# brownvc/matryodshka

Measured on AMD Instinct MI355X. Metric: novel-view frames/sec, 640x320 ODS->32-sphere MSI infer+render, higher is better.
Workload: dtype f32

## Files before the change

### matryodshka_amd/csrc/cnn_x3.hip

```cpp
#include "cnn_device.h"

namespace {

#ifndef MSI_X3_EARLY_DMA
#define MSI_X3_EARLY_DMA 0
#endif
#ifndef MSI_X3_NSTG
#define MSI_X3_NSTG 0
#endif
#ifndef MSI_X3_ABLATE
#define MSI_X3_ABLATE 0
#endif
#ifndef MSI_X2_NSTG
#define MSI_X2_NSTG 3
#endif
constexpr int x3_rate_y(int RATE) { return RATE == 3 ? 1 : RATE; }
constexpr int x3_rate_x(int RATE) { return RATE == 3 ? 2 : RATE; }
constexpr int x3_nstg(int RATE, int NPL) { return NPL == 2 ? MSI_X2_NSTG : (MSI_X3_NSTG ? MSI_X3_NSTG : (RATE == 2 ? 3 : 2)); }
template <int RATE, int NS = x3_nstg(RATE, 3), int NPL = 3, int TH = 4>
struct HaloGeomX3 {
  static constexpr int PW = 16 + 2 * x3_rate_x(RATE), PH = TH + 2 * x3_rate_y(RATE), NPX = PW * PH;
  static constexpr int PIX_BYTES = NPL * 64 + 16;
  static constexpr int ROW_PITCH = ((PW * PIX_BYTES + 127) / 256) * 256 + 128;
  static constexpr int A_BYTES = PH * ROW_PITCH;
  static constexpr int B_ROW = 64;
  static constexpr int B_PLANE = 64 * B_ROW, B_STAGE = NPL * B_PLANE;
  static constexpr int NSTG = NS;
  static constexpr int LDS_BYTES = A_BYTES + NSTG * B_STAGE;
  static constexpr int NLOAD = (NPX * 8 + 255) / 256;
};
__device__ __forceinline__ void f16_range_track(unsigned &amax, v4f y) {
  const float fx = y.x, fy = y.y, fz = y.z, fw = y.w;
  const unsigned a = __builtin_bit_cast(unsigned, fx) & 0x7fffffffu, b = __builtin_bit_cast(unsigned, fy) & 0x7fffffffu;
  const unsigned c = __builtin_bit_cast(unsigned, fz) & 0x7fffffffu, d = __builtin_bit_cast(unsigned, fw) & 0x7fffffffu;
  amax = max(max(amax, a), max(b, max(c, d)));
}
constexpr unsigned F16_MAX_BITS = 0x477fe000u;

template <int N>
__device__ __forceinline__ void wait_lgkm4(v4f &a, v4f &b, v4f &c, v4f &d) {
  asm volatile("s_waitcnt lgkmcnt(%4)" : "+v"(a), "+v"(b), "+v"(c), "+v"(d) : "n"(N) : "memory");
}
template <int N>
__device__ __forceinline__ void wait_lgkm6(v4f &a, v4f &b, v4f &c, v4f &d, v4f &e, v4f &f) {
  asm volatile("s_waitcnt lgkmcnt(%6)" : "+v"(a), "+v"(b), "+v"(c), "+v"(d), "+v"(e), "+v"(f) : "n"(N) : "memory");
}

#ifndef MSI_X2_WAVES
#define MSI_X2_WAVES 4
#endif
#ifndef MSI_X2_LATE_CB
#define MSI_X2_LATE_CB 1
#endif
template <int NP>
__device__ __forceinline__ void split_mfma(f32x16 &acc, f32x16 &lo, const v4f &ah, const v4f &am, const v4f &al, const v4f &bh, const v4f &bm, const v4f &bl);
template <int RATE, int APPLY, int NPL, int TH>
__device__ __forceinline__ void conv_halo_x3_body(const ConvParams &p, char *smem) {
  typedef HaloGeomX3<RATE, x3_nstg(RATE, NPL), NPL, TH> G;
  constexpr int RY = x3_rate_y(RATE), RX = x3_rate_x(RATE), PW = G::PW, NPX = G::NPX, NLOAD = G::NLOAD;
  static_assert(RATE != 3 || TH == 4, "row-parity tiles: four rows");
  constexpr int MT = TH / 4, NT = 1, BM = 16 * TH;
  static_assert(TH == 4 || (TH == 8 && NPL == 3 && RATE == 1), "the 8-row tile is built for the six-product form at rate 1");
#ifdef MSI_CONV_TIMING
  const unsigned long long ts0 = __builtin_amdgcn_s_memtime(), ts0r = __builtin_amdgcn_s_memrealtime();
#endif
  const int tid = threadIdx.x, lane = tid & 63;
  const int wave = __builtin_amdgcn_readfirstlane(tid >> 6);
  const int wm = wave >> 1, wn = wave & 1;
  const int CH = p.cpt0;
  int t, c0 = 0, c1 = CH, ks = 0, slot = 0;
  {
    const int bid = blockIdx.x;
    if (bid < p.nb_main && p.split0 == 1) {
      const int q = p.n_main >> 3, r = p.n_main & 7, xcd = bid & 7, local = bid >> 3;
      t = (xcd < r ? xcd * (q + 1) : r * (q + 1) + (xcd - r) * q) + local;
    } else {
      int sp, r, tbase;
      unsigned mg;
      if (bid < p.nb_main) { sp = p.split0; mg = p.mg_sp0; r = bid; tbase = 0; }
      else { sp = p.split; mg = p.mg_sp; r = bid - p.nb_main; tbase = p.n_main; }
      const int tl = (int)udiv_magic((unsigned)r, (unsigned)sp, mg);
      ks = r - tl * sp;
      t = tbase + tl;
      c0 = (int)udiv_magic((unsigned)(ks * CH), (unsigned)sp, mg);
      c1 = (int)udiv_magic((unsigned)((ks + 1) * CH), (unsigned)sp, mg);
      slot = bid - (p.split0 == 1 ? p.nb_main : 0);
    }
  }
  const bool full = (c0 == 0) & (c1 == CH);
  int tile_m, tile_n, b;
  {
    int r = t;
    const int q1 = (int)udiv_magic((unsigned)r, (unsigned)p.tiles_m, p.mg_tm);
    tile_m = r - q1 * p.tiles_m; r = q1;
    const int q2 = (int)udiv_magic((unsigned)r, (unsigned)p.tiles_n, p.mg_tn);
    tile_n = r - q2 * p.tiles_n;
    b = q2;
  }
  LnShard shard = {0, 0};
  if (APPLY) shard = ln_shard_load(p.ln_sums + (size_t)b * LN_SHARDS * LN_WORDS, tid);
  const int tyi = (int)udiv_magic((unsigned)tile_m, (unsigned)p.halo_tx, p.mg_htx);
  const int ow0 = (tile_m - tyi * p.halo_tx) * 16;
  const int H = p.Hin, W = p.Win, C = p.C0;
  v4f cbv[4] = {};
  if (MT == 1 && (!MSI_X2_LATE_CB || NPL != 2)) load_coord_bias(p, tile_m, tile_n, tid, cbv);
  const int S = p.ksteps;
  const int plane_bytes = p.npad * G::B_ROW;
  const __amdgpu_buffer_rsrc_t rsrc_b = __builtin_amdgcn_make_buffer_rsrc((void *)p.wpk_x3, 0, (int)((size_t)S * NPL * plane_bytes), 0x00020000);
  const unsigned b_voff = (unsigned)((tile_n * 64 + wave * 16 + (lane >> 2)) * G::B_ROW + (lane & 3) * 16);
  int c = c0, cpar = 0;
  (void)cpar;
  auto b_issue = [&](const int c, const int tap, const int st) __attribute__((always_inline)) {
    if (MSI_X3_ABLATE & 1) return;
    char *sB_ = smem + G::A_BYTES + st * G::B_STAGE + wave * 16 * G::B_ROW;
    const int soff_ = (tap * CH + c) * NPL * plane_bytes;
    __builtin_amdgcn_raw_ptr_buffer_load_lds(rsrc_b, (lds_void *)sB_, 16, b_voff, soff_, 0, 0);
    __builtin_amdgcn_raw_ptr_buffer_load_lds(rsrc_b, (lds_void *)(sB_ + G::B_PLANE), 16, b_voff, soff_ + plane_bytes, 0, 0);
    if (NPL == 3) __builtin_amdgcn_raw_ptr_buffer_load_lds(rsrc_b, (lds_void *)(sB_ + 2 * G::B_PLANE), 16, b_voff, soff_ + 2 * plane_bytes, 0, 0);
  };
  b_issue(c0, 0, 0);
  if (G::NSTG == 3) b_issue(c0, 1, 1);

  unsigned voff[NLOAD], lds_a[NLOAD];
  bool pok[NLOAD];
  const int cslot = tid & 7;
#pragma unroll
  for (int k = 0; k < NLOAD; ++k) {
    const int pp = (tid + 256 * k) >> 3;
    const int py = pp / PW, px = pp - py * PW;
    const int ih = RATE == 3 ? (tyi >> 1) * (2 * TH) + (tyi & 1) + 2 * (py - 1) : tyi * TH - RY + py;
    int iw = ow0 - RX + px;
    if (p.wrap) iw = iw < 0 ? iw + W : (iw >= W ? iw - W : iw);
    pok[k] = pp < NPX && ih >= 0 && ih < H && iw >= 0 && iw < W;
    voff[k] = pok[k] ? __umul24((unsigned)(ih * W + iw), (unsigned)(C * 4)) + (unsigned)(cslot * 16) : OOB;
    lds_a[k] = pp < NPX ? (unsigned)(py * G::ROW_PITCH + px * G::PIX_BYTES + cslot * 8) : 0xffffffffu;
  }
  const size_t in_bytes = (size_t)H * W * C * 4;
  const __amdgpu_buffer_rsrc_t rsrc_a = __builtin_amdgcn_make_buffer_rsrc((void *)(p.x0 + (size_t)b * in_bytes), 0, (int)in_bytes, 0x00020000);

  float inv_f = 1.f, mu_hi = 0.f, mu_lo = 0.f;
  bool has_pad = false;
  if (APPLY) {
    bool bad = false;
#pragma unroll
    for (int k = 0; k < NLOAD; ++k) bad |= (lds_a[k] != 0xffffffffu) && !pok[k];
    has_pad = __builtin_amdgcn_ballot_w64(bad) != 0;
  }
  v4f araw[NLOAD], g4, be4;
  unsigned amax_ = 0u;
  auto patch_load = [&](const int c) __attribute__((always_inline)) {
#pragma unroll
    for (int k_ = 0; k_ < NLOAD; ++k_)
      araw[k_] = __builtin_bit_cast(v4f, (u32x4_t)__builtin_amdgcn_raw_buffer_load_b128(rsrc_a, voff[k_], c * ROW_BYTES, 0));
    if (APPLY) {
      g4 = *reinterpret_cast<const v4f *>(p.ln_gamma + c * 32 + cslot * 4);
      be4 = *reinterpret_cast<const v4f *>(p.ln_beta + c * 32 + cslot * 4);
    }
  };
  auto patch_store = [&]() __attribute__((always_inline)) {
    v4f s4 = {1.f, 1.f, 1.f, 1.f}, t4 = {0.f, 0.f, 0.f, 0.f};
    if (APPLY) {
      s4 = inv_f * g4;
      const v4f nh = {-mu_hi, -mu_hi, -mu_hi, -mu_hi}, nl = {-mu_lo, -mu_lo, -mu_lo, -mu_lo};
      t4 = __builtin_elementwise_fma(nl, s4, __builtin_elementwise_fma(nh, s4, be4));
    }
#pragma unroll
    for (int k_ = 0; k_ < NLOAD; ++k_) {
      v4f y = araw[k_];
      if (APPLY) {
        y = __builtin_elementwise_max(__builtin_elementwise_fma(y, s4, t4), v4f{0.f, 0.f, 0.f, 0.f});
        if (has_pad && !pok[k_]) y = v4f{0.f, 0.f, 0.f, 0.f};
      }
      if (NPL == 2) {
        typedef _Float16 h2_t __attribute__((ext_vector_type(2)));
        typedef unsigned u2x_t __attribute__((ext_vector_type(2)));
        f16_range_track(amax_, y);
        const h2_t ha = {(_Float16)y.x, (_Float16)y.y}, hb = {(_Float16)y.z, (_Float16)y.w};
        const h2_t ma = {(_Float16)((y.x - (float)ha.x) * 2048.f), (_Float16)((y.y - (float)ha.y) * 2048.f)};
        const h2_t mb = {(_Float16)((y.z - (float)hb.x) * 2048.f), (_Float16)((y.w - (float)hb.y) * 2048.f)};
        if (lds_a[k_] != 0xffffffffu) {
          *reinterpret_cast<u2x_t *>(smem + lds_a[k_]) = u2x_t{__builtin_bit_cast(unsigned, ha), __builtin_bit_cast(unsigned, hb)};
          *reinterpret_cast<u2x_t *>(smem + lds_a[k_] + 64) = u2x_t{__builtin_bit_cast(unsigned, ma), __builtin_bit_cast(unsigned, mb)};
        }
      } else {
      unsigned h0, h1, m0, m1, l0, l1;
      asm("v_cvt_pk_bf16_f32 %0, %1, %2" : "=v"(h0) : "v"(y.x), "v"(y.y));
      asm("v_cvt_pk_bf16_f32 %0, %1, %2" : "=v"(h1) : "v"(y.z), "v"(y.w));
      v4f r = y - v4f{__builtin_bit_cast(float, h0 << 16), __builtin_bit_cast(float, h0 & 0xffff0000u),
                      __builtin_bit_cast(float, h1 << 16), __builtin_bit_cast(float, h1 & 0xffff0000u)};
      asm("v_cvt_pk_bf16_f32 %0, %1, %2" : "=v"(m0) : "v"(r.x), "v"(r.y));
      asm("v_cvt_pk_bf16_f32 %0, %1, %2" : "=v"(m1) : "v"(r.z), "v"(r.w));
      r = r - v4f{__builtin_bit_cast(float, m0 << 16), __builtin_bit_cast(float, m0 & 0xffff0000u),
                  __builtin_bit_cast(float, m1 << 16), __builtin_bit_cast(float, m1 & 0xffff0000u)};
      asm("v_cvt_pk_bf16_f32 %0, %1, %2" : "=v"(l0) : "v"(r.x), "v"(r.y));
      asm("v_cvt_pk_bf16_f32 %0, %1, %2" : "=v"(l1) : "v"(r.z), "v"(r.w));
      if (lds_a[k_] != 0xffffffffu) {
        typedef unsigned u2x_t __attribute__((ext_vector_type(2)));
        *reinterpret_cast<u2x_t *>(smem + lds_a[k_]) = u2x_t{h0, h1};
        *reinterpret_cast<u2x_t *>(smem + lds_a[k_] + 64) = u2x_t{m0, m1};
        *reinterpret_cast<u2x_t *>(smem + lds_a[k_] + 128) = u2x_t{l0, l1};
      }
    }
    }
  };
  const int frow = lane & 31, fh = lane >> 5, fswz = (frow >> 1) & 7;
  const unsigned lds_base = (unsigned)(size_t)(lds_void *)smem;
  const unsigned a_base = lds_base + (unsigned)((2 * MT * wm + (frow >> 4)) * G::ROW_PITCH + ((frow & 15) ^ ((frow >> 4) << 3)) * G::PIX_BYTES + fh * 16);
  unsigned b_s[2];
  (void)fswz;
#pragma unroll
  for (int s_ = 0; s_ < 2; ++s_)
    b_s[s_] = lds_base + G::A_BYTES + (wn * 32 + frow) * G::B_ROW + (((2 * s_ + fh) ^ ((frow >> 2) & 3)) << 4);
  typedef __bf16 bf16x8 __attribute__((ext_vector_type(8)));
  typedef _Float16 f16x8 __attribute__((ext_vector_type(8)));
  f32x16 acc[MT][1], acc_lo;
#pragma unroll
  for (int i = 0; i < MT; ++i)
#pragma unroll
    for (int r = 0; r < 16; ++r) acc[i][0][r] = acc_lo[r] = 0.f;

  auto htap = [&](auto TAP_c) __attribute__((always_inline)) {
    constexpr int TAP = decltype(TAP_c)::value;
    constexpr int KH_ = TAP / 3, KW_ = TAP % 3;
    const unsigned bst_ = (unsigned)(G::NSTG == 3 ? TAP % 3 : ((TAP ^ cpar) & 1)) * G::B_STAGE;
    constexpr int AOFF_ = KH_ * RY * G::ROW_PITCH + KW_ * RX * G::PIX_BYTES;
    v4f ah_[2], am_[2], al_[2], bh_[2], bm_[2], bl_[2];
    if (MSI_X3_EARLY_DMA || G::NSTG == 2) {
      constexpr int PD_ = G::NSTG - 1;
      const int stn_ = G::NSTG == 3 ? (TAP + 2) % 3 : (((TAP ^ cpar) & 1) ^ 1);
      if (TAP + PD_ < 9) { b_issue(c, TAP + PD_, stn_); }
      else if (c + 1 < c1) { b_issue(c + 1, TAP + PD_ - 9, stn_); }
    }
    if (NPL == 2) {
#pragma unroll
      for (int s_ = 0; s_ < 2; ++s_) {
        ah_[s_] = s_ == 0 ? lds_read128<AOFF_>(a_base) : lds_read128<AOFF_ + 32>(a_base);
        bh_[s_] = lds_read128<0>(b_s[s_] + bst_);
        am_[s_] = s_ == 0 ? lds_read128<AOFF_ + 64>(a_base) : lds_read128<AOFF_ + 96>(a_base);
        bm_[s_] = lds_read128<G::B_PLANE>(b_s[s_] + bst_);
      }
#pragma unroll
      for (int s_ = 0; s_ < 2; ++s_) {
        if (s_ == 0) wait_lgkm4<4>(ah_[0], bh_[0], am_[0], bm_[0]);
        else wait_lgkm4<0>(ah_[1], bh_[1], am_[1], bm_[1]);
        acc_lo = __builtin_amdgcn_mfma_f32_32x32x16_f16(__builtin_bit_cast(f16x8, bm_[s_]), __builtin_bit_cast(f16x8, ah_[s_]), acc_lo, 0, 0, 0);
        acc[0][0] = __builtin_amdgcn_mfma_f32_32x32x16_f16(__builtin_bit_cast(f16x8, bh_[s_]), __builtin_bit_cast(f16x8, ah_[s_]), acc[0][0], 0, 0, 0);
        acc_lo = __builtin_amdgcn_mfma_f32_32x32x16_f16(__builtin_bit_cast(f16x8, bh_[s_]), __builtin_bit_cast(f16x8, am_[s_]), acc_lo, 0, 0, 0);
        __builtin_amdgcn_sched_barrier(0);
        if (s_ == 0) {
          if (TAP == 0 && c + 1 < c1) patch_load(c + 1);
          if (!MSI_X3_EARLY_DMA && G::NSTG == 3) {
            if (TAP + 2 < 9) { b_issue(c, TAP + 2, (TAP + 2) % 3); }
            else if (c + 1 < c1) { b_issue(c + 1, TAP - 7, (TAP + 2) % 3); }
          }
        }
      }
    } else if constexpr (MT == 2) {
      constexpr int A1_ = AOFF_ + 2 * G::ROW_PITCH;
      v4f xh_[2][2], xm_[2][2], xl_[2][2];
      bh_[0] = lds_read128<0>(b_s[0] + bst_); bm_[0] = lds_read128<G::B_PLANE>(b_s[0] + bst_); bl_[0] = lds_read128<2 * G::B_PLANE>(b_s[0] + bst_);
      xh_[0][0] = lds_read128<AOFF_>(a_base); xm_[0][0] = lds_read128<AOFF_ + 64>(a_base); xl_[0][0] = lds_read128<AOFF_ + 128>(a_base);
      xh_[0][1] = lds_read128<A1_>(a_base); xm_[0][1] = lds_read128<A1_ + 64>(a_base); xl_[0][1] = lds_read128<A1_ + 128>(a_base);
      bh_[1] = lds_read128<0>(b_s[1] + bst_); bm_[1] = lds_read128<G::B_PLANE>(b_s[1] + bst_); bl_[1] = lds_read128<2 * G::B_PLANE>(b_s[1] + bst_);
      wait_lgkm6<6>(bh_[0], bm_[0], bl_[0], xh_[0][0], xm_[0][0], xl_[0][0]);
      split_mfma<3>(acc[0][0], acc_lo, xh_[0][0], xm_[0][0], xl_[0][0], bh_[0], bm_[0], bl_[0]);
      __builtin_amdgcn_sched_barrier(0);
      xh_[1][0] = lds_read128<AOFF_ + 32>(a_base); xm_[1][0] = lds_read128<AOFF_ + 96>(a_base); xl_[1][0] = lds_read128<AOFF_ + 160>(a_base);
      xh_[1][1] = lds_read128<A1_ + 32>(a_base); xm_[1][1] = lds_read128<A1_ + 96>(a_base); xl_[1][1] = lds_read128<A1_ + 160>(a_base);
      if (TAP == 0 && c + 1 < c1) patch_load(c + 1);
      wait_lgkm6<9>(xh_[0][1], xm_[0][1], xl_[0][1], bh_[0], bm_[0], bl_[0]);
      split_mfma<3>(acc[1][0], acc_lo, xh_[0][1], xm_[0][1], xl_[0][1], bh_[0], bm_[0], bl_[0]);
      __builtin_amdgcn_sched_barrier(0);
      wait_lgkm6<3>(bh_[1], bm_[1], bl_[1], xh_[1][0], xm_[1][0], xl_[1][0]);
      split_mfma<3>(acc[0][0], acc_lo, xh_[1][0], xm_[1][0], xl_[1][0], bh_[1], bm_[1], bl_[1]);
      __builtin_amdgcn_sched_barrier(0);
      wait_lgkm6<0>(xh_[1][1], xm_[1][1], xl_[1][1], bh_[1], bm_[1], bl_[1]);
      split_mfma<3>(acc[1][0], acc_lo, xh_[1][1], xm_[1][1], xl_[1][1], bh_[1], bm_[1], bl_[1]);
      __builtin_amdgcn_sched_barrier(0);
    } else {
    if (!(MSI_X3_ABLATE & 8))
#pragma unroll
      for (int s_ = 0; s_ < 2; ++s_) {
      ah_[s_] = s_ == 0 ? lds_read128<AOFF_>(a_base) : lds_read128<AOFF_ + 32>(a_base);
      bh_[s_] = lds_read128<0>(b_s[s_] + bst_);
      am_[s_] = s_ == 0 ? lds_read128<AOFF_ + 64>(a_base) : lds_read128<AOFF_ + 96>(a_base);
      bm_[s_] = lds_read128<G::B_PLANE>(b_s[s_] + bst_);
      al_[s_] = s_ == 0 ? lds_read128<AOFF_ + 128>(a_base) : lds_read128<AOFF_ + 160>(a_base);
      bl_[s_] = lds_read128<2 * G::B_PLANE>(b_s[s_] + bst_);
    }
#pragma unroll
      for (int s_ = 0; s_ < 2; ++s_) {
      if (s_ == 0) wait_lgkm6<6>(ah_[0], bh_[0], am_[0], bm_[0], al_[0], bl_[0]);
      else wait_lgkm6<0>(ah_[1], bh_[1], am_[1], bm_[1], al_[1], bl_[1]);
      if (!(MSI_X3_ABLATE & 16)) {
      acc[0][0] = __builtin_amdgcn_mfma_f32_32x32x16_bf16(__builtin_bit_cast(bf16x8, bm_[s_]), __builtin_bit_cast(bf16x8, am_[s_]), acc[0][0], 0, 0, 0);
      acc[0][0] = __builtin_amdgcn_mfma_f32_32x32x16_bf16(__builtin_bit_cast(bf16x8, bh_[s_]), __builtin_bit_cast(bf16x8, al_[s_]), acc[0][0], 0, 0, 0);
      acc[0][0] = __builtin_amdgcn_mfma_f32_32x32x16_bf16(__builtin_bit_cast(bf16x8, bl_[s_]), __builtin_bit_cast(bf16x8, ah_[s_]), acc[0][0], 0, 0, 0);
      acc[0][0] = __builtin_amdgcn_mfma_f32_32x32x16_bf16(__builtin_bit_cast(bf16x8, bh_[s_]), __builtin_bit_cast(bf16x8, am_[s_]), acc[0][0], 0, 0, 0);
      acc[0][0] = __builtin_amdgcn_mfma_f32_32x32x16_bf16(__builtin_bit_cast(bf16x8, bm_[s_]), __builtin_bit_cast(bf16x8, ah_[s_]), acc[0][0], 0, 0, 0);
      acc[0][0] = __builtin_amdgcn_mfma_f32_32x32x16_bf16(__builtin_bit_cast(bf16x8, bh_[s_]), __builtin_bit_cast(bf16x8, ah_[s_]), acc[0][0], 0, 0, 0);
      }
      __builtin_amdgcn_sched_barrier(0);
      if (s_ == 0) {
        if (TAP == 0 && c + 1 < c1) patch_load(c + 1);
        if (!MSI_X3_EARLY_DMA && G::NSTG == 3) {
        if (TAP + 2 < 9) { b_issue(c, TAP + 2, (TAP + 2) % 3); }
        else if (c + 1 < c1) { b_issue(c + 1, TAP - 7, (TAP + 2) % 3); }
        }
      }
    }
    }
    {
      const bool issued_ = (TAP + 2 < 9) || (c + 1 < c1);
      if (G::NSTG == 2) {
        if (TAP == 0 && c + 1 < c1) wait_vmcnt<NLOAD + (APPLY ? 2 : 0)>();
        else wait_vmcnt<0>();
      } else if (TAP == 0 && c + 1 < c1) wait_vmcnt<NPL + NLOAD + (APPLY ? 2 : 0)>();
      else if (issued_) wait_vmcnt<NPL>();
      else wait_vmcnt<0>();
    }
    if (!(MSI_X3_ABLATE & 4)) __builtin_amdgcn_s_barrier();
  };

  patch_load(c0);
  if (APPLY) {
    double *s_stat = reinterpret_cast<double *>(smem);
    ln_mean_inv_pre(shard, p.ln_inv_n, p.ln_scl_src, p.status, s_stat, tid);
    const double mu = s_stat[0];
    inv_f = (float)s_stat[1];
    mu_hi = (float)mu;
    mu_lo = (float)(mu - (double)mu_hi);
    __syncthreads();
  }
  wait_vmcnt<0>();
  patch_store();
  asm volatile("s_waitcnt lgkmcnt(0)" ::: "memory");
  __builtin_amdgcn_s_barrier();
#ifdef MSI_CONV_TIMING
  const unsigned long long ts1 = __builtin_amdgcn_s_memtime();
#endif
  for (; c < c1; ++c) {
    cpar = (c - c0) & 1;
    htap(IC<0>{}); htap(IC<1>{}); htap(IC<2>{}); htap(IC<3>{}); htap(IC<4>{}); htap(IC<5>{}); htap(IC<6>{}); htap(IC<7>{}); htap(IC<8>{});
    if (c + 1 < c1 && !(MSI_X3_ABLATE & 32)) {
      patch_store();
      asm volatile("s_waitcnt lgkmcnt(0)" ::: "memory");
      __builtin_amdgcn_s_barrier();
    }
  }
  if (MSI_X2_LATE_CB && NPL == 2) load_coord_bias(p, tile_m, tile_n, tid, cbv);
  if (NPL == 2) {
#pragma unroll
    for (int r = 0; r < 16; ++r) acc[0][0][r] = __builtin_fmaf(acc_lo[r], 1.f / 2048.f, acc[0][0][r]);
    if (__builtin_amdgcn_ballot_w64(amax_ > F16_MAX_BITS) != 0 && lane == 0) atomicOr(p.status, STATUS_F16_SPLIT_RANGE);
  }

#ifdef MSI_CONV_TIMING
  const unsigned long long ts2 = __builtin_amdgcn_s_memtime();
  auto stamp = [&]() __attribute__((always_inline)) {
    if (p.dbg && tid == 0) {
      unsigned long long *o = p.dbg + (size_t)blockIdx.x * 24;
      o[0] = ts0; o[1] = ts1; o[2] = ts2; o[3] = __builtin_amdgcn_s_memtime(); o[22] = ts0r; o[23] = __builtin_amdgcn_s_memrealtime();
      o[4] = __builtin_amdgcn_s_getreg(4 | (31 << 11));
      o[5] = __builtin_amdgcn_s_getreg(20 | (31 << 11));
    }
  };
#endif
  if (!full) {
    constexpr int SLAB = BM * 64 * 4;
    const __amdgpu_buffer_rsrc_t rsrc_p = __builtin_amdgcn_make_buffer_rsrc((void *)(p.partial + (size_t)slot * (BM * 64)), 0, SLAB, 0x00020000);
    if (p.tile_cnt == nullptr) {
      dump_acc<MT, NT, 0>(acc, rsrc_p, tid);
#ifdef MSI_CONV_TIMING
      stamp();
#endif
      return;
    }
    dump_acc<MT, NT, MSI_HANDOFF_AUX>(acc, rsrc_p, tid);
    const int nsp = t < p.n_main ? p.split0 : p.split;
    asm volatile("s_waitcnt vmcnt(0)" ::: "memory");
    handoff_release();
    __syncthreads();
    int *s_old = reinterpret_cast<int *>(smem);
    if (tid == 0)
      *s_old = __hip_atomic_fetch_add(p.tile_cnt + (t - (p.split0 == 1 ? p.n_main : 0)), 1, __ATOMIC_RELAXED, __HIP_MEMORY_SCOPE_AGENT);
    __syncthreads();
    if (*s_old != nsp - 1) return;
    handoff_acquire();
    const __amdgpu_buffer_rsrc_t rsrc_t = __builtin_amdgcn_make_buffer_rsrc((void *)(p.partial + (size_t)(slot - ks) * (BM * 64)), 0, nsp * SLAB, 0x00020000);
    sum_slabs<MT, NT, MSI_HANDOFF_AUX>(acc, rsrc_t, nsp, SLAB, tid);
    __syncthreads();
  }
  emit_tile<BM, 64, MODE_CONV>(p, acc, tile_m, tile_n, 0, b, tid, cbv, MT == 1 && p.coord_bias != nullptr, smem);
#ifdef MSI_CONV_TIMING
  stamp();
#endif
}

template <int RATE, int APPLY, int NPL>
__global__ void __launch_bounds__(256) __attribute__((amdgpu_waves_per_eu((NPL == 2 && RATE == 1) ? MSI_X2_WAVES : 2)))
conv_halo_x3_kernel(const ConvParams p) {
#if defined(__HIP_DEVICE_COMPILE__)
  extern __shared__ __attribute__((aligned(16))) char smem[];
  conv_halo_x3_body<RATE, APPLY, NPL, 4>(p, smem);
#endif
}
template <int APPLY, int NPL>
__global__ void __launch_bounds__(256) __attribute__((amdgpu_waves_per_eu(2)))
conv_halo8_x3_kernel(const ConvParams p) {
#if defined(__HIP_DEVICE_COMPILE__)
  extern __shared__ __attribute__((aligned(16))) char smem[];
  conv_halo_x3_body<1, APPLY, NPL, 8>(p, smem);
#endif
}

template <int NP>
__device__ __forceinline__ void split_store(char *smem, unsigned off, v4f y, unsigned &amax) {
  typedef unsigned u2x_t __attribute__((ext_vector_type(2)));
  if (NP == 2) {
    typedef _Float16 h2_t __attribute__((ext_vector_type(2)));
    f16_range_track(amax, y);
    const h2_t ha = {(_Float16)y.x, (_Float16)y.y}, hb = {(_Float16)y.z, (_Float16)y.w};
    const h2_t ma = {(_Float16)((y.x - (float)ha.x) * 2048.f), (_Float16)((y.y - (float)ha.y) * 2048.f)};
    const h2_t mb = {(_Float16)((y.z - (float)hb.x) * 2048.f), (_Float16)((y.w - (float)hb.y) * 2048.f)};
    if (off != 0xffffffffu) {
      *reinterpret_cast<u2x_t *>(smem + off) = u2x_t{__builtin_bit_cast(unsigned, ha), __builtin_bit_cast(unsigned, hb)};
      *reinterpret_cast<u2x_t *>(smem + off + 64) = u2x_t{__builtin_bit_cast(unsigned, ma), __builtin_bit_cast(unsigned, mb)};
    }
  } else {
    unsigned h0, h1, m0, m1, l0, l1;
    asm("v_cvt_pk_bf16_f32 %0, %1, %2" : "=v"(h0) : "v"(y.x), "v"(y.y));
    asm("v_cvt_pk_bf16_f32 %0, %1, %2" : "=v"(h1) : "v"(y.z), "v"(y.w));
    v4f r = y - v4f{__builtin_bit_cast(float, h0 << 16), __builtin_bit_cast(float, h0 & 0xffff0000u),
                    __builtin_bit_cast(float, h1 << 16), __builtin_bit_cast(float, h1 & 0xffff0000u)};
    asm("v_cvt_pk_bf16_f32 %0, %1, %2" : "=v"(m0) : "v"(r.x), "v"(r.y));
    asm("v_cvt_pk_bf16_f32 %0, %1, %2" : "=v"(m1) : "v"(r.z), "v"(r.w));
    r = r - v4f{__builtin_bit_cast(float, m0 << 16), __builtin_bit_cast(float, m0 & 0xffff0000u),
                __builtin_bit_cast(float, m1 << 16), __builtin_bit_cast(float, m1 & 0xffff0000u)};
    asm("v_cvt_pk_bf16_f32 %0, %1, %2" : "=v"(l0) : "v"(r.x), "v"(r.y));
    asm("v_cvt_pk_bf16_f32 %0, %1, %2" : "=v"(l1) : "v"(r.z), "v"(r.w));
    if (off != 0xffffffffu) {
      *reinterpret_cast<u2x_t *>(smem + off) = u2x_t{h0, h1};
      *reinterpret_cast<u2x_t *>(smem + off + 64) = u2x_t{m0, m1};
      *reinterpret_cast<u2x_t *>(smem + off + 128) = u2x_t{l0, l1};
    }
  }
}
template <int NP>
__device__ __forceinline__ void split_mfma(f32x16 &acc, f32x16 &lo, const v4f &ah, const v4f &am, const v4f &al, const v4f &bh, const v4f &bm, const v4f &bl) {
  typedef __bf16 bf16x8 __attribute__((ext_vector_type(8)));
  typedef _Float16 f16x8 __attribute__((ext_vector_type(8)));
  if (NP == 2) {
    lo = __builtin_amdgcn_mfma_f32_32x32x16_f16(__builtin_bit_cast(f16x8, bm), __builtin_bit_cast(f16x8, ah), lo, 0, 0, 0);
    acc = __builtin_amdgcn_mfma_f32_32x32x16_f16(__builtin_bit_cast(f16x8, bh), __builtin_bit_cast(f16x8, ah), acc, 0, 0, 0);
    lo = __builtin_amdgcn_mfma_f32_32x32x16_f16(__builtin_bit_cast(f16x8, bh), __builtin_bit_cast(f16x8, am), lo, 0, 0, 0);
  } else {
    acc = __builtin_amdgcn_mfma_f32_32x32x16_bf16(__builtin_bit_cast(bf16x8, bm), __builtin_bit_cast(bf16x8, am), acc, 0, 0, 0);
    acc = __builtin_amdgcn_mfma_f32_32x32x16_bf16(__builtin_bit_cast(bf16x8, bh), __builtin_bit_cast(bf16x8, al), acc, 0, 0, 0);
    acc = __builtin_amdgcn_mfma_f32_32x32x16_bf16(__builtin_bit_cast(bf16x8, bl), __builtin_bit_cast(bf16x8, ah), acc, 0, 0, 0);
    acc = __builtin_amdgcn_mfma_f32_32x32x16_bf16(__builtin_bit_cast(bf16x8, bh), __builtin_bit_cast(bf16x8, am), acc, 0, 0, 0);
    acc = __builtin_amdgcn_mfma_f32_32x32x16_bf16(__builtin_bit_cast(bf16x8, bm), __builtin_bit_cast(bf16x8, ah), acc, 0, 0, 0);
    acc = __builtin_amdgcn_mfma_f32_32x32x16_bf16(__builtin_bit_cast(bf16x8, bh), __builtin_bit_cast(bf16x8, ah), acc, 0, 0, 0);
  }
}
template <int NP>
__device__ __forceinline__ void split_finish(f32x16 &acc, const f32x16 &lo, unsigned amax, int lane, int *status) {
  if (NP == 2) {
#pragma unroll
    for (int r = 0; r < 16; ++r) acc[r] = __builtin_fmaf(lo[r], 1.f / 2048.f, acc[r]);
    if (__builtin_amdgcn_ballot_w64(amax > F16_MAX_BITS) != 0 && lane == 0) atomicOr(status, STATUS_F16_SPLIT_RANGE);
  }
}

#ifndef MSI_S2X3_NSTG
#define MSI_S2X3_NSTG 2
#endif
template <int NP, int TH = 4>
struct HaloGeomS2X3 {
  static constexpr int PW = 17, PH = TH + 1, NPX = PW * PH;
  static constexpr int PIX_BYTES = NP * 64 + 16;
  static constexpr int ROW_PITCH = ((PW * PIX_BYTES + 127) / 256) * 256 + 128;
  static constexpr int A_BYTES = PH * ROW_PITCH;
  static constexpr int B_ROW = 64, B_PLANE = 64 * B_ROW, B_STAGE = NP * B_PLANE;
// ... 603 lines not shown

  if (!full) {
    constexpr int SLAB = BM * 64 * 4;
    if (p.tile_cnt == nullptr) {
#pragma unroll
      for (int cl = 0; cl < 2; ++cl) {
        const __amdgpu_buffer_rsrc_t rsrc_p = __builtin_amdgcn_make_buffer_rsrc((void *)(p.partial + ((size_t)slot * 2 + cl) * (BM * 64)), 0, SLAB, 0x00020000);
        dump_acc<MT, 1, 0>(acc[cl], rsrc_p, tid);
      }
      return;
    }
#pragma unroll
    for (int cl = 0; cl < 2; ++cl) {
      const __amdgpu_buffer_rsrc_t rsrc_p = __builtin_amdgcn_make_buffer_rsrc((void *)(p.partial + ((size_t)slot * 2 + cl) * (BM * 64)), 0, SLAB, 0x00020000);
      dump_acc<MT, 1, MSI_HANDOFF_AUX>(acc[cl], rsrc_p, tid);
    }
    const int nsp = t < p.n_main ? p.split0 : p.split;
    asm volatile("s_waitcnt vmcnt(0)" ::: "memory");
    handoff_release();
    __syncthreads();
    int *s_old = reinterpret_cast<int *>(smem);
    if (tid == 0)
      *s_old = __hip_atomic_fetch_add(p.tile_cnt + (t - (p.split0 == 1 ? p.n_main : 0)), 1, __ATOMIC_RELAXED, __HIP_MEMORY_SCOPE_AGENT);
    __syncthreads();
    if (*s_old != nsp - 1) return;
    handoff_acquire();
#pragma unroll
    for (int cl = 0; cl < 2; ++cl) {
      const __amdgpu_buffer_rsrc_t rsrc_t = __builtin_amdgcn_make_buffer_rsrc((void *)(p.partial + ((size_t)(slot - ks) * 2 + cl) * (BM * 64)), 0, nsp * 2 * SLAB, 0x00020000);
      sum_slabs<MT, 1, MSI_HANDOFF_AUX>(acc[cl], rsrc_t, nsp, 2 * SLAB, tid);
    }
  }
#pragma unroll
  for (int cl = 0; cl < 2; ++cl) emit_tile<BM, 64, MODE_CONVT>(p, acc[cl], tile_m, tile_n, 2 * ph + cl, b, tid);
}

template <int NP>
__global__ void __launch_bounds__(256) __attribute__((amdgpu_waves_per_eu(2, MSI_CT_MAXW)))
convt_halo_x3_kernel(const ConvParams p) {
#if defined(__HIP_DEVICE_COMPILE__)
  extern __shared__ __attribute__((aligned(16))) char smem[];
  convt_halo_x3_body<NP, 4>(p, smem);
#endif
}

__global__ void __launch_bounds__(256) __attribute__((amdgpu_waves_per_eu(2)))
convt_halo8_x3_kernel(const ConvParams p) {
#if defined(__HIP_DEVICE_COMPILE__)
  extern __shared__ __attribute__((aligned(16))) char smem[];
  convt_halo_x3_body<3, 8>(p, smem);
#endif
}

}

namespace msi_cnn {
int launch_x3(const LayerLaunch &Q, const ConvParams &p, int rate, hipStream_t stream) {
  const dim3 grid(Q.nblocks), block(256);
  if (Q.halo_t) {
    constexpr int lds_ct3 = HaloGeomCT3<MSI_CT3_NSTG, 3>::LDS_BYTES, lds_ct2 = HaloGeomCT3<3, 2>::LDS_BYTES;
    constexpr int lds_ct8 = HaloGeomCT3<MSI_CT3_NSTG, 3, 8>::LDS_BYTES;
    static_assert(lds_ct8 <= 65536, "convt_halo8_x3_kernel: LDS without the launch attribute");
    if (Q.x3_th8) hipLaunchKernelGGL(convt_halo8_x3_kernel, grid, block, lds_ct8, stream, p);
    else if (Q.halo_x2) hipLaunchKernelGGL(convt_halo_x3_kernel<2>, grid, block, lds_ct2, stream, p);
    else hipLaunchKernelGGL(convt_halo_x3_kernel<3>, grid, block, lds_ct3, stream, p);
    int rc = msi::check_launch("convt_halo_x3");
    if (!rc && Q.nfix > 0 && p.tile_cnt == nullptr) rc = launch_fixup(Q.x3_th8 ? 128 : 64, 64, MODE_CONVT, Q.nfix, 2, p, stream);
    return rc;
  }
  if (Q.halo_s2 && Q.x3_th8) {
    typedef HaloGeomS2X3<3, 8> G8s_;
    static_assert(G8s_::LDS_BYTES <= 65536, "conv_halo8_s2_x3_kernel: LDS without the launch attribute");
    if (Q.halo_apply) hipLaunchKernelGGL((conv_halo8_s2_x3_kernel<1>), grid, block, G8s_::LDS_BYTES, stream, p);
    else hipLaunchKernelGGL((conv_halo8_s2_x3_kernel<0>), grid, block, G8s_::LDS_BYTES, stream, p);
  } else if (Q.halo_s2) {
    if (Q.halo_x2) {
      if (Q.halo_apply) hipLaunchKernelGGL((conv_halo_s2_x3_kernel<1, 2>), grid, block, HaloGeomS2X3<2>::LDS_BYTES, stream, p);
      else hipLaunchKernelGGL((conv_halo_s2_x3_kernel<0, 2>), grid, block, HaloGeomS2X3<2>::LDS_BYTES, stream, p);
    } else {
      if (Q.halo_apply) hipLaunchKernelGGL((conv_halo_s2_x3_kernel<1, 3>), grid, block, HaloGeomS2X3<3>::LDS_BYTES, stream, p);
      else hipLaunchKernelGGL((conv_halo_s2_x3_kernel<0, 3>), grid, block, HaloGeomS2X3<3>::LDS_BYTES, stream, p);
    }
  } else if (Q.x3_th8) {
    typedef HaloGeomX3<1, (MSI_X3_NSTG ? MSI_X3_NSTG : 2), 3, 8> G8_;
    static_assert(G8_::LDS_BYTES <= 65536, "conv_halo8_x3_kernel: LDS without the launch attribute");
    if (Q.halo_apply) hipLaunchKernelGGL((conv_halo8_x3_kernel<1, 3>), grid, block, G8_::LDS_BYTES, stream, p);
    else hipLaunchKernelGGL((conv_halo8_x3_kernel<0, 3>), grid, block, G8_::LDS_BYTES, stream, p);
  } else {
    static thread_local unsigned long long done2[12] = {0};
#define MSI_X3_LAUNCH(R, A, N)                                                                                         \
  {                                                                                                                    \
    typedef HaloGeomX3<R, x3_nstg(R, N), N> G_;                                                                        \
    if (G_::LDS_BYTES > 65536) {                                                                                       \
      int rc0 = set_max_lds(reinterpret_cast<const void *>(conv_halo_x3_kernel<R, A, N>), G_::LDS_BYTES, done2[(R - 1) * 4 + A * 2 + (N - 2)], "conv_halo_x3"); \
      if (rc0) return rc0;                                                                                             \
    }                                                                                                                  \
    hipLaunchKernelGGL((conv_halo_x3_kernel<R, A, N>), grid, block, G_::LDS_BYTES, stream, p);                          \
  }
    const int sel = (rate == 1 ? 0 : (p.row_par ? 8 : 4)) + (Q.halo_apply ? 2 : 0) + (Q.halo_x2 ? 0 : 1);
    switch (sel) {
      case 0: MSI_X3_LAUNCH(1, 0, 2) break;
      case 1: MSI_X3_LAUNCH(1, 0, 3) break;
      case 2: MSI_X3_LAUNCH(1, 1, 2) break;
      case 3: MSI_X3_LAUNCH(1, 1, 3) break;
      case 4: MSI_X3_LAUNCH(2, 0, 2) break;
      case 5: MSI_X3_LAUNCH(2, 0, 3) break;
      case 6: MSI_X3_LAUNCH(2, 1, 2) break;
      case 7: MSI_X3_LAUNCH(2, 1, 3) break;
      case 8: MSI_X3_LAUNCH(3, 0, 2) break;
      case 9: MSI_X3_LAUNCH(3, 0, 3) break;
      case 10: MSI_X3_LAUNCH(3, 1, 2) break;
      default: MSI_X3_LAUNCH(3, 1, 3) break;
    }
#undef MSI_X3_LAUNCH
  }
  int rc = msi::check_launch("conv_halo_x3");
  if (!rc && Q.nfix > 0 && p.tile_cnt == nullptr) rc = launch_fixup(Q.x3_th8 ? 128 : 64, 64, MODE_CONV, Q.nfix, 1, p, stream);
  return rc;
}
}
```

Before: 551.0.

## Software-pipeline LDS fragment reads and weight DMA across taps in 3-plane halo conv

```diff
diff --git a/matryodshka_amd/csrc/cnn_x3.hip b/matryodshka_amd/csrc/cnn_x3.hip
--- a/matryodshka_amd/csrc/cnn_x3.hip
+++ b/matryodshka_amd/csrc/cnn_x3.hip
@@ -8,6 +8,9 @@
 #ifndef MSI_X3_NSTG
 #define MSI_X3_NSTG 0
 #endif
+#ifndef MSI_X3_NSTG8
+#define MSI_X3_NSTG8 2
+#endif
 #ifndef MSI_X3_ABLATE
 #define MSI_X3_ABLATE 0
 #endif
@@ -16,7 +19,7 @@
 #endif
 constexpr int x3_rate_y(int RATE) { return RATE == 3 ? 1 : RATE; }
 constexpr int x3_rate_x(int RATE) { return RATE == 3 ? 2 : RATE; }
-constexpr int x3_nstg(int RATE, int NPL) { return NPL == 2 ? MSI_X2_NSTG : (MSI_X3_NSTG ? MSI_X3_NSTG : (RATE == 2 ? 3 : 2)); }
+constexpr int x3_nstg(int RATE, int NPL, int TH = 4) { return NPL == 2 ? MSI_X2_NSTG : (TH == 8 ? MSI_X3_NSTG8 : (MSI_X3_NSTG ? MSI_X3_NSTG : 3)); }
 template <int RATE, int NS = x3_nstg(RATE, 3), int NPL = 3, int TH = 4>
 struct HaloGeomX3 {
   static constexpr int PW = 16 + 2 * x3_rate_x(RATE), PH = TH + 2 * x3_rate_y(RATE), NPX = PW * PH;
@@ -46,6 +49,15 @@
   asm volatile("s_waitcnt lgkmcnt(%6)" : "+v"(a), "+v"(b), "+v"(c), "+v"(d), "+v"(e), "+v"(f) : "n"(N) : "memory");
 }
 
+template <int N>
+__device__ __forceinline__ void wait_lgkm3x2(v4f (&a)[3], v4f (&b)[3]) {
+  asm volatile("s_waitcnt lgkmcnt(%6)" : "+v"(a[0]), "+v"(a[1]), "+v"(a[2]), "+v"(b[0]), "+v"(b[1]), "+v"(b[2]) : "n"(N) : "memory");
+}
+template <int N>
+__device__ __forceinline__ void wait_lgkm3x3(v4f (&a)[3], v4f (&b)[3], v4f (&c)[3]) {
+  asm volatile("s_waitcnt lgkmcnt(%9)" : "+v"(a[0]), "+v"(a[1]), "+v"(a[2]), "+v"(b[0]), "+v"(b[1]), "+v"(b[2]), "+v"(c[0]), "+v"(c[1]), "+v"(c[2]) : "n"(N) : "memory");
+}
+
 #ifndef MSI_X2_WAVES
 #define MSI_X2_WAVES 4
 #endif
@@ -56,7 +68,7 @@
 __device__ __forceinline__ void split_mfma(f32x16 &acc, f32x16 &lo, const v4f &ah, const v4f &am, const v4f &al, const v4f &bh, const v4f &bm, const v4f &bl);
 template <int RATE, int APPLY, int NPL, int TH>
 __device__ __forceinline__ void conv_halo_x3_body(const ConvParams &p, char *smem) {
-  typedef HaloGeomX3<RATE, x3_nstg(RATE, NPL), NPL, TH> G;
+  typedef HaloGeomX3<RATE, x3_nstg(RATE, NPL, TH), NPL, TH> G;
   constexpr int RY = x3_rate_y(RATE), RX = x3_rate_x(RATE), PW = G::PW, NPX = G::NPX, NLOAD = G::NLOAD;
   static_assert(RATE != 3 || TH == 4, "row-parity tiles: four rows");
   constexpr int MT = TH / 4, NT = 1, BM = 16 * TH;
@@ -119,7 +131,8 @@
     if (NPL == 3) __builtin_amdgcn_raw_ptr_buffer_load_lds(rsrc_b, (lds_void *)(sB_ + 2 * G::B_PLANE), 16, b_voff, soff_ + 2 * plane_bytes, 0, 0);
   };
   b_issue(c0, 0, 0);
-  if (G::NSTG == 3) b_issue(c0, 1, 1);
+  if (G::NSTG == 3 || NPL == 3) b_issue(c0, 1, 1);
+  if (G::NSTG == 3 && NPL == 3) b_issue(c0, 2, 2);
 
   unsigned voff[NLOAD], lds_a[NLOAD];
   bool pok[NLOAD];
@@ -224,91 +237,35 @@
     constexpr int KH_ = TAP / 3, KW_ = TAP % 3;
     const unsigned bst_ = (unsigned)(G::NSTG == 3 ? TAP % 3 : ((TAP ^ cpar) & 1)) * G::B_STAGE;
     constexpr int AOFF_ = KH_ * RY * G::ROW_PITCH + KW_ * RX * G::PIX_BYTES;
-    v4f ah_[2], am_[2], al_[2], bh_[2], bm_[2], bl_[2];
+    v4f ah_[2], am_[2], bh_[2], bm_[2];
     if (MSI_X3_EARLY_DMA || G::NSTG == 2) {
       constexpr int PD_ = G::NSTG - 1;
       const int stn_ = G::NSTG == 3 ? (TAP + 2) % 3 : (((TAP ^ cpar) & 1) ^ 1);
       if (TAP + PD_ < 9) { b_issue(c, TAP + PD_, stn_); }
       else if (c + 1 < c1) { b_issue(c + 1, TAP + PD_ - 9, stn_); }
     }
-    if (NPL == 2) {
-#pragma unroll
-      for (int s_ = 0; s_ < 2; ++s_) {
-        ah_[s_] = s_ == 0 ? lds_read128<AOFF_>(a_base) : lds_read128<AOFF_ + 32>(a_base);
-        bh_[s_] = lds_read128<0>(b_s[s_] + bst_);
-        am_[s_] = s_ == 0 ? lds_read128<AOFF_ + 64>(a_base) : lds_read128<AOFF_ + 96>(a_base);
-        bm_[s_] = lds_read128<G::B_PLANE>(b_s[s_] + bst_);
-      }
-#pragma unroll
-      for (int s_ = 0; s_ < 2; ++s_) {
-        if (s_ == 0) wait_lgkm4<4>(ah_[0], bh_[0], am_[0], bm_[0]);
-        else wait_lgkm4<0>(ah_[1], bh_[1], am_[1], bm_[1]);
-        acc_lo = __builtin_amdgcn_mfma_f32_32x32x16_f16(__builtin_bit_cast(f16x8, bm_[s_]), __builtin_bit_cast(f16x8, ah_[s_]), acc_lo, 0, 0, 0);
-        acc[0][0] = __builtin_amdgcn_mfma_f32_32x32x16_f16(__builtin_bit_cast(f16x8, bh_[s_]), __builtin_bit_cast(f16x8, ah_[s_]), acc[0][0], 0, 0, 0);
-        acc_lo = __builtin_amdgcn_mfma_f32_32x32x16_f16(__builtin_bit_cast(f16x8, bh_[s_]), __builtin_bit_cast(f16x8, am_[s_]), acc_lo, 0, 0, 0);
-        __builtin_amdgcn_sched_barrier(0);
-        if (s_ == 0) {
-          if (TAP == 0 && c + 1 < c1) patch_load(c + 1);
-          if (!MSI_X3_EARLY_DMA && G::NSTG == 3) {
-            if (TAP + 2 < 9) { b_issue(c, TAP + 2, (TAP + 2) % 3); }
-            else if (c + 1 < c1) { b_issue(c + 1, TAP - 7, (TAP + 2) % 3); }
-          }
-        }
-      }
-    } else if constexpr (MT == 2) {
-      constexpr int A1_ = AOFF_ + 2 * G::ROW_PITCH;
-      v4f xh_[2][2], xm_[2][2], xl_[2][2];
-      bh_[0] = lds_read128<0>(b_s[0] + bst_); bm_[0] = lds_read128<G::B_PLANE>(b_s[0] + bst_); bl_[0] = lds_read128<2 * G::B_PLANE>(b_s[0] + bst_);
-      xh_[0][0] = lds_read128<AOFF_>(a_base); xm_[0][0] = lds_read128<AOFF_ + 64>(a_base); xl_[0][0] = lds_read128<AOFF_ + 128>(a_base);
-      xh_[0][1] = lds_read128<A1_>(a_base); xm_[0][1] = lds_read128<A1_ + 64>(a_base); xl_[0][1] = lds_read128<A1_ + 128>(a_base);
-      bh_[1] = lds_read128<0>(b_s[1] + bst_); bm_[1] = lds_read128<G::B_PLANE>(b_s[1] + bst_); bl_[1] = lds_read128<2 * G::B_PLANE>(b_s[1] + bst_);
-      wait_lgkm6<6>(bh_[0], bm_[0], bl_[0], xh_[0][0], xm_[0][0], xl_[0][0]);
-      split_mfma<3>(acc[0][0], acc_lo, xh_[0][0], xm_[0][0], xl_[0][0], bh_[0], bm_[0], bl_[0]);
-      __builtin_amdgcn_sched_barrier(0);
-      xh_[1][0] = lds_read128<AOFF_ + 32>(a_base); xm_[1][0] = lds_read128<AOFF_ + 96>(a_base); xl_[1][0] = lds_read128<AOFF_ + 160>(a_base);
-      xh_[1][1] = lds_read128<A1_ + 32>(a_base); xm_[1][1] = lds_read128<A1_ + 96>(a_base); xl_[1][1] = lds_read128<A1_ + 160>(a_base);
-      if (TAP == 0 && c + 1 < c1) patch_load(c + 1);
-      wait_lgkm6<9>(xh_[0][1], xm_[0][1], xl_[0][1], bh_[0], bm_[0], bl_[0]);
-      split_mfma<3>(acc[1][0], acc_lo, xh_[0][1], xm_[0][1], xl_[0][1], bh_[0], bm_[0], bl_[0]);
-      __builtin_amdgcn_sched_barrier(0);
-      wait_lgkm6<3>(bh_[1], bm_[1], bl_[1], xh_[1][0], xm_[1][0], xl_[1][0]);
-      split_mfma<3>(acc[0][0], acc_lo, xh_[1][0], xm_[1][0], xl_[1][0], bh_[1], bm_[1], bl_[1]);
-      __builtin_amdgcn_sched_barrier(0);
-      wait_lgkm6<0>(xh_[1][1], xm_[1][1], xl_[1][1], bh_[1], bm_[1], bl_[1]);
-      split_mfma<3>(acc[1][0], acc_lo, xh_[1][1], xm_[1][1], xl_[1][1], bh_[1], bm_[1], bl_[1]);
-      __builtin_amdgcn_sched_barrier(0);
-    } else {
-    if (!(MSI_X3_ABLATE & 8))
-#pragma unroll
-      for (int s_ = 0; s_ < 2; ++s_) {
+#pragma unroll
+    for (int s_ = 0; s_ < 2; ++s_) {
       ah_[s_] = s_ == 0 ? lds_read128<AOFF_>(a_base) : lds_read128<AOFF_ + 32>(a_base);
       bh_[s_] = lds_read128<0>(b_s[s_] + bst_);
       am_[s_] = s_ == 0 ? lds_read128<AOFF_ + 64>(a_base) : lds_read128<AOFF_ + 96>(a_base);
       bm_[s_] = lds_read128<G::B_PLANE>(b_s[s_] + bst_);
-      al_[s_] = s_ == 0 ? lds_read128<AOFF_ + 128>(a_base) : lds_read128<AOFF_ + 160>(a_base);
-      bl_[s_] = lds_read128<2 * G::B_PLANE>(b_s[s_] + bst_);
-    }
-#pragma unroll
-      for (int s_ = 0; s_ < 2; ++s_) {
-      if (s_ == 0) wait_lgkm6<6>(ah_[0], bh_[0], am_[0], bm_[0], al_[0], bl_[0]);
-      else wait_lgkm6<0>(ah_[1], bh_[1], am_[1], bm_[1], al_[1], bl_[1]);
-      if (!(MSI_X3_ABLATE & 16)) {
-      acc[0][0] = __builtin_amdgcn_mfma_f32_32x32x16_bf16(__builtin_bit_cast(bf16x8, bm_[s_]), __builtin_bit_cast(bf16x8, am_[s_]), acc[0][0], 0, 0, 0);
-      acc[0][0] = __builtin_amdgcn_mfma_f32_32x32x16_bf16(__builtin_bit_cast(bf16x8, bh_[s_]), __builtin_bit_cast(bf16x8, al_[s_]), acc[0][0], 0, 0, 0);
-      acc[0][0] = __builtin_amdgcn_mfma_f32_32x32x16_bf16(__builtin_bit_cast(bf16x8, bl_[s_]), __builtin_bit_cast(bf16x8, ah_[s_]), acc[0][0], 0, 0, 0);
-      acc[0][0] = __builtin_amdgcn_mfma_f32_32x32x16_bf16(__builtin_bit_cast(bf16x8, bh_[s_]), __builtin_bit_cast(bf16x8, am_[s_]), acc[0][0], 0, 0, 0);
-      acc[0][0] = __builtin_amdgcn_mfma_f32_32x32x16_bf16(__builtin_bit_cast(bf16x8, bm_[s_]), __builtin_bit_cast(bf16x8, ah_[s_]), acc[0][0], 0, 0, 0);
-      acc[0][0] = __builtin_amdgcn_mfma_f32_32x32x16_bf16(__builtin_bit_cast(bf16x8, bh_[s_]), __builtin_bit_cast(bf16x8, ah_[s_]), acc[0][0], 0, 0, 0);
-      }
+    }
+#pragma unroll
+    for (int s_ = 0; s_ < 2; ++s_) {
+      if (s_ == 0) wait_lgkm4<4>(ah_[0], bh_[0], am_[0], bm_[0]);
+      else wait_lgkm4<0>(ah_[1], bh_[1], am_[1], bm_[1]);
+      acc_lo = __builtin_amdgcn_mfma_f32_32x32x16_f16(__builtin_bit_cast(f16x8, bm_[s_]), __builtin_bit_cast(f16x8, ah_[s_]), acc_lo, 0, 0, 0);
+      acc[0][0] = __builtin_amdgcn_mfma_f32_32x32x16_f16(__builtin_bit_cast(f16x8, bh_[s_]), __builtin_bit_cast(f16x8, ah_[s_]), acc[0][0], 0, 0, 0);
+      acc_lo = __builtin_amdgcn_mfma_f32_32x32x16_f16(__builtin_bit_cast(f16x8, bh_[s_]), __builtin_bit_cast(f16x8, am_[s_]), acc_lo, 0, 0, 0);
       __builtin_amdgcn_sched_barrier(0);
       if (s_ == 0) {
         if (TAP == 0 && c + 1 < c1) patch_load(c + 1);
         if (!MSI_X3_EARLY_DMA && G::NSTG == 3) {
-        if (TAP + 2 < 9) { b_issue(c, TAP + 2, (TAP + 2) % 3); }
-        else if (c + 1 < c1) { b_issue(c + 1, TAP - 7, (TAP + 2) % 3); }
+          if (TAP + 2 < 9) { b_issue(c, TAP + 2, (TAP + 2) % 3); }
+          else if (c + 1 < c1) { b_issue(c + 1, TAP - 7, (TAP + 2) % 3); }
         }
       }
-    }
     }
     {
       const bool issued_ = (TAP + 2 < 9) || (c + 1 < c1);
@@ -320,6 +277,99 @@
       else wait_vmcnt<0>();
     }
     if (!(MSI_X3_ABLATE & 4)) __builtin_amdgcn_s_barrier();
+  };
+
+  v4f fa_[2][MT][2][3], fb_[2][2][3];
+  auto rd_x = [&](auto TAP_c, auto I_c, auto S_c) __attribute__((always_inline)) {
+    constexpr int T_ = decltype(TAP_c)::value, I_ = decltype(I_c)::value, S_ = decltype(S_c)::value;
+    constexpr int O_ = (T_ / 3) * RY * G::ROW_PITCH + (T_ % 3) * RX * G::PIX_BYTES + I_ * 2 * G::ROW_PITCH + S_ * 32;
+    if (MSI_X3_ABLATE & 8) return;
+    fa_[T_ & 1][I_][S_][0] = lds_read128<O_>(a_base); fa_[T_ & 1][I_][S_][1] = lds_read128<O_ + 64>(a_base); fa_[T_ & 1][I_][S_][2] = lds_read128<O_ + 128>(a_base);
+  };
+  auto rd_x1 = [&](auto TAP_c, auto I_c, auto S_c, auto P_c) __attribute__((always_inline)) {
+    constexpr int T_ = decltype(TAP_c)::value, I_ = decltype(I_c)::value, S_ = decltype(S_c)::value, P_ = decltype(P_c)::value;
+    constexpr int O_ = (T_ / 3) * RY * G::ROW_PITCH + (T_ % 3) * RX * G::PIX_BYTES + I_ * 2 * G::ROW_PITCH + S_ * 32 + P_ * 64;
+    if (MSI_X3_ABLATE & 8) return;
+    fa_[T_ & 1][I_][S_][P_] = lds_read128<O_>(a_base);
+  };
+  auto stage_of = [&](auto TAP_c) __attribute__((always_inline)) {
+    constexpr int T_ = decltype(TAP_c)::value;
+    return G::NSTG == 3 ? T_ % 3 : ((T_ ^ cpar) & 1);
+  };
+  auto rd_w1 = [&](auto TAP_c, auto S_c, auto P_c) __attribute__((always_inline)) {
+    constexpr int T_ = decltype(TAP_c)::value, S_ = decltype(S_c)::value, P_ = decltype(P_c)::value;
+    if (MSI_X3_ABLATE & 8) return;
+    fb_[T_ & 1][S_][P_] = lds_read128<P_ * G::B_PLANE>(b_s[S_] + (unsigned)stage_of(TAP_c) * G::B_STAGE);
+  };
+  auto rd_w = [&](auto TAP_c, auto S_c) __attribute__((always_inline)) { rd_w1(TAP_c, S_c, IC<0>{}); rd_w1(TAP_c, S_c, IC<1>{}); rd_w1(TAP_c, S_c, IC<2>{}); };
+  auto dma1 = [&](auto TAP_c, auto P_c) __attribute__((always_inline)) {
+    constexpr int T_ = decltype(TAP_c)::value + G::NSTG, P_ = decltype(P_c)::value;
+    if (MSI_X3_ABLATE & 1) return;
+    if (T_ >= 9 && !(c + 1 < c1)) return;
+    char *sB_ = smem + G::A_BYTES + stage_of(TAP_c) * G::B_STAGE + wave * 16 * G::B_ROW + P_ * G::B_PLANE;
+    const int soff_ = ((T_ % 9) * CH + (T_ < 9 ? c : c + 1)) * NPL * plane_bytes + P_ * plane_bytes;
+    __builtin_amdgcn_raw_ptr_buffer_load_lds(rsrc_b, (lds_void *)sB_, 16, b_voff, soff_, 0, 0);
+  };
+  auto mgroup = [&](f32x16 &a_, const v4f (&x_)[3], const v4f (&w_)[3], auto fill_) __attribute__((always_inline)) {
+#define MSI_X3_MFMA(K, W, X)                                                                                                                        \
+    if (!(MSI_X3_ABLATE & 16)) a_ = __builtin_amdgcn_mfma_f32_32x32x16_bf16(__builtin_bit_cast(bf16x8, w_[W]), __builtin_bit_cast(bf16x8, x_[X]), a_, 0, 0, 0); \
+    fill_(IC<K>{});                                                                                                                                 \
+    __builtin_amdgcn_sched_barrier(0);
+    MSI_X3_MFMA(0, 1, 1) MSI_X3_MFMA(1, 0, 2) MSI_X3_MFMA(2, 2, 0) MSI_X3_MFMA(3, 0, 1) MSI_X3_MFMA(4, 1, 0) MSI_X3_MFMA(5, 0, 0)
+#undef MSI_X3_MFMA
+  };
+  auto ptap = [&](auto TAP_c) __attribute__((always_inline)) {
+    constexpr int TAP = decltype(TAP_c)::value, CS = TAP & 1;
+    constexpr bool PRE = TAP < 8;
+    typedef IC<(TAP + 1) % 9> NX;
+    typedef IC<0> I0; typedef IC<1> I1; typedef IC<2> I2;
+    const bool more_ = c + 1 < c1;
+    if constexpr (TAP == 0) {
+      rd_x(TAP_c, I0{}, I0{});
+      if constexpr (MT == 2) rd_x(TAP_c, I1{}, I0{}); else rd_x(TAP_c, I0{}, I1{});
+      rd_w(TAP_c, I0{}); rd_w(TAP_c, I1{});
+      wait_lgkm3x2<3>(fa_[CS][0][0], fb_[CS][0]);
+      if constexpr (MT == 2) { rd_x(TAP_c, I0{}, I1{}); rd_x(TAP_c, I1{}, I1{}); }
+    } else {
+      wait_lgkm3x2<MT == 2 ? 9 : 3>(fa_[CS][0][0], fb_[CS][0]);
+    }
+    __builtin_amdgcn_sched_barrier(0);
+    mgroup(acc[0][0], fa_[CS][0][0], fb_[CS][0], [&](auto K_c) __attribute__((always_inline)) {
+      constexpr int K_ = decltype(K_c)::value;
+      if constexpr (PRE) { if constexpr (MT == 2) rd_x1(NX{}, IC<K_ / 3>{}, I0{}, IC<K_ % 3>{}); else rd_x1(NX{}, I0{}, IC<K_ / 3>{}, IC<K_ % 3>{}); }
+    });
+    if constexpr (MT == 2) wait_lgkm3x3<PRE ? 6 : 0>(fb_[CS][1], fa_[CS][0][1], fa_[CS][MT - 1][1]);
+    else wait_lgkm3x2<PRE ? 6 : 0>(fb_[CS][1], fa_[CS][0][1]);
+    {
+      constexpr int PL_ = NLOAD + (APPLY ? 2 : 0);
+      constexpr bool pl_ = TAP >= 1 && TAP <= G::NSTG - 1;
+      if (G::NSTG == 2) {
+        if (pl_ && more_) wait_vmcnt<PL_>(); else wait_vmcnt<0>();
+      } else {
+        if (TAP + 2 < 9 || more_) { if (pl_ && more_) wait_vmcnt<NPL + PL_>(); else wait_vmcnt<NPL>(); }
+        else wait_vmcnt<0>();
+      }
+    }
+    if (!(MSI_X3_ABLATE & 4)) __builtin_amdgcn_s_barrier();
+    __builtin_amdgcn_sched_barrier(0);
+    auto fill_w = [&](auto K_c) __attribute__((always_inline)) {
+      constexpr int K_ = decltype(K_c)::value;
+      if (K_ % 2 == 0) dma1(TAP_c, IC<K_ / 2>{});
+      if constexpr (PRE) rd_w1(NX{}, IC<K_ / 3>{}, IC<K_ % 3>{});
+    };
+    if constexpr (MT == 2) {
+      mgroup(acc[1][0], fa_[CS][1][0], fb_[CS][0], fill_w);
+      if constexpr (PRE) wait_lgkm3x3<6>(fb_[CS][1], fa_[CS][0][1], fa_[CS][1][1]);
+      mgroup(acc[0][0], fa_[CS][0][1], fb_[CS][1], [&](auto K_c) __attribute__((always_inline)) {
+        constexpr int K_ = decltype(K_c)::value;
+        if constexpr (PRE) rd_x1(NX{}, IC<K_ / 3>{}, I1{}, IC<K_ % 3>{});
+      });
+      if (TAP == 0 && more_) { patch_load(c + 1); __builtin_amdgcn_sched_barrier(0); }
+      mgroup(acc[1][0], fa_[CS][1][1], fb_[CS][1], [&](auto) __attribute__((always_inline)) {});
+    } else {
+      mgroup(acc[0][0], fa_[CS][0][1], fb_[CS][1], fill_w);
+      if (TAP == 0 && more_) { patch_load(c + 1); __builtin_amdgcn_sched_barrier(0); }
+    }
   };
 
   patch_load(c0);
@@ -341,7 +391,8 @@
 #endif
   for (; c < c1; ++c) {
     cpar = (c - c0) & 1;
-    htap(IC<0>{}); htap(IC<1>{}); htap(IC<2>{}); htap(IC<3>{}); htap(IC<4>{}); htap(IC<5>{}); htap(IC<6>{}); htap(IC<7>{}); htap(IC<8>{});
+    if constexpr (NPL == 3) { ptap(IC<0>{}); ptap(IC<1>{}); ptap(IC<2>{}); ptap(IC<3>{}); ptap(IC<4>{}); ptap(IC<5>{}); ptap(IC<6>{}); ptap(IC<7>{}); ptap(IC<8>{}); }
+    else { htap(IC<0>{}); htap(IC<1>{}); htap(IC<2>{}); htap(IC<3>{}); htap(IC<4>{}); htap(IC<5>{}); htap(IC<6>{}); htap(IC<7>{}); htap(IC<8>{}); }
     if (c + 1 < c1 && !(MSI_X3_ABLATE & 32)) {
       patch_store();
       asm volatile("s_waitcnt lgkmcnt(0)" ::: "memory");
@@ -398,7 +449,7 @@
 }
 
 template <int RATE, int APPLY, int NPL>
-__global__ void __launch_bounds__(256) __attribute__((amdgpu_waves_per_eu((NPL == 2 && RATE == 1) ? MSI_X2_WAVES : 2)))
+__global__ void __launch_bounds__(256) __attribute__((amdgpu_waves_per_eu((NPL == 2 && RATE == 1) ? MSI_X2_WAVES : ((NPL == 3 && x3_nstg(RATE, NPL) == 2) ? 3 : 2))))
 conv_halo_x3_kernel(const ConvParams p) {
 #if defined(__HIP_DEVICE_COMPILE__)
   extern __shared__ __attribute__((aligned(16))) char smem[];
@@ -1168,8 +1219,13 @@
       else hipLaunchKernelGGL((conv_halo_s2_x3_kernel<0, 3>), grid, block, HaloGeomS2X3<3>::LDS_BYTES, stream, p);
     }
   } else if (Q.x3_th8) {
-    typedef HaloGeomX3<1, (MSI_X3_NSTG ? MSI_X3_NSTG : 2), 3, 8> G8_;
-    static_assert(G8_::LDS_BYTES <= 65536, "conv_halo8_x3_kernel: LDS without the launch attribute");
+    typedef HaloGeomX3<1, x3_nstg(1, 3, 8), 3, 8> G8_;
+    if (G8_::LDS_BYTES > 65536) {
+      static thread_local unsigned long long done8[2] = {0};
+      int rc0 = Q.halo_apply ? set_max_lds(reinterpret_cast<const void *>(conv_halo8_x3_kernel<1, 3>), G8_::LDS_BYTES, done8[1], "conv_halo8_x3")
+                             : set_max_lds(reinterpret_cast<const void *>(conv_halo8_x3_kernel<0, 3>), G8_::LDS_BYTES, done8[0], "conv_halo8_x3");
+      if (rc0) return rc0;
+    }
     if (Q.halo_apply) hipLaunchKernelGGL((conv_halo8_x3_kernel<1, 3>), grid, block, G8_::LDS_BYTES, stream, p);
     else hipLaunchKernelGGL((conv_halo8_x3_kernel<0, 3>), grid, block, G8_::LDS_BYTES, stream, p);
   } else {
```

Result: no change. 547.0, median of 2 (-0.7%).
